# nerficg-project/faster-gaussian-splatting

Hardware: AMD Instinct MI355X
Metric: train_iters_per_sec (higher is better)
Workload: dtype f32; 1 GPU; S2: 3000000 garden-like Gaussians (SH degree 3), 1920x1080, 8 orbit views; full training iteration fwd+loss+bwd+Adam (BASELINE.json configs[2]), loss 0.8*L1+0.2*DSSIM, densification_info updated; parallelism=single GPU, n_gaussians=3000000, active_sh_bases=16, forward=one host read per pass (fgs_forward), world=1, backend=none (single process), device=cuda:0 (AMD Radeon Graphics)

## Files before the change

### faster-gaussian-splatting_amd/csrc/adam.hip

```cpp
#include "fgs_adam.h"

namespace fgs {


template <bool NT> __device__ __forceinline__ float4 load4(const float* p) { return NT ? load_float4_nt(p) : *reinterpret_cast<const float4*>(p); }
template <bool NT> __device__ __forceinline__ void store4(float* p, const float4 v) {
    if (NT) store_float4_nt(p, v);
    else *reinterpret_cast<float4*>(p) = v;
}

__device__ __forceinline__ bool adam_block_gradient_needed(const AdamArgs& a, const AdamGroup& G, const uint32_t b) {
    if (a.live_blocks[b] != 0) return true;
    return !(G.grad[(size_t)b * 64u * G.row_len] == 0.0f);
}

enum : int { kAdamSkip = 0, kAdamZero = 1, kAdamRead = 2 };
__device__ __forceinline__ int adam_piece_plan(const AdamArgs& a, const AdamGroup& G, const int64_t first, const int64_t last) {
    if (a.live_blocks == nullptr || G.row_len == 0u) return kAdamRead;
    const uint32_t r0 = static_cast<uint32_t>(first) / G.row_len, r1 = static_cast<uint32_t>(last) / G.row_len;
    const uint32_t b0 = r0 >> 6, b1 = r1 >> 6;
    const bool need0 = adam_block_gradient_needed(a, G, b0), need1 = b1 == b0 ? need0 : adam_block_gradient_needed(a, G, b1);
    if (a.quiet_blocks != nullptr) {
        const uint8_t q0 = a.quiet_blocks[b0], q1 = b1 == b0 ? q0 : a.quiet_blocks[b1];
        if (need0 && q0 != 0) a.quiet_blocks[b0] = 0;
        if (b1 != b0 && need1 && q1 != 0) a.quiet_blocks[b1] = 0;
        if (!need0 && !need1 && q0 != 0 && q1 != 0) return kAdamSkip;
    }
    return need0 || need1 ? kAdamRead : kAdamZero;
}

template <int U, bool NT>
__global__ void __launch_bounds__(256) adam_kernel(const AdamArgs a) {
    const uint32_t blk = a.reverse ? a.total_blocks - 1u - blockIdx.x : blockIdx.x;
    int gidx = 0;
#pragma unroll
    for (int j = 1; j < 8; ++j) if (j < a.n_groups && blk >= a.g[j].first_block) gidx = j;
    const AdamGroup& G = a.g[gidx];
    const int64_t block_base = (int64_t)(blk - G.first_block) * (256 * 4 * U);
    float4 g4[U];
    float4 p4[U], m4[U], v4[U];
    bool full[U], run[U];
#pragma unroll
    for (int u = 0; u < U; ++u) {
        const int64_t base = block_base + ((int64_t)u * 256 + threadIdx.x) * 4;
        full[u] = base + 4 <= G.n;
        run[u] = false;
        if (full[u]) {
            const int plan = adam_piece_plan(a, G, base, base + 3);
            run[u] = plan != kAdamSkip;
            if (run[u]) {
                g4[u] = plan == kAdamRead ? load4<NT>(G.grad + base) : make_float4(0.0f, 0.0f, 0.0f, 0.0f);
                p4[u] = load4<NT>(G.param + base); m4[u] = load4<NT>(G.exp_avg + base); v4[u] = load4<NT>(G.exp_avg_sq + base);
            }
        }
    }
#pragma unroll
    for (int u = 0; u < U; ++u) {
        const int64_t base = block_base + ((int64_t)u * 256 + threadIdx.x) * 4;
        if (full[u]) {
            if (run[u]) {
                adam_update(p4[u].x, m4[u].x, v4[u].x, g4[u].x, G.h); adam_update(p4[u].y, m4[u].y, v4[u].y, g4[u].y, G.h);
                adam_update(p4[u].z, m4[u].z, v4[u].z, g4[u].z, G.h); adam_update(p4[u].w, m4[u].w, v4[u].w, g4[u].w, G.h);
                store4<NT>(G.param + base, p4[u]); store4<NT>(G.exp_avg + base, m4[u]); store4<NT>(G.exp_avg_sq + base, v4[u]);
            }
        } else if (base < G.n) {
            const int plan = adam_piece_plan(a, G, base, G.n - 1);
            if (plan != kAdamSkip)
                adam_scalar_tail(G.param, G.exp_avg, G.exp_avg_sq, base, G.n, G.h, [&](const int64_t e) { return plan == kAdamRead ? G.grad[e] : 0.0f; });
        }
    }
}

__global__ void __launch_bounds__(256) adam_quiet_scan_kernel(const AdamQuietScanArgs a) {
    const uint32_t b = blockIdx.x;
    const uint32_t rows = min(64u, a.rows - b * 64u);
    bool zero = true;
    for (int k = 0; k < a.n_groups; ++k) {
        const size_t first = (size_t)b * 64u * a.row_len[k];
        const uint32_t len = rows * a.row_len[k];
#pragma unroll
        for (int w = 0; w < 2; ++w) {
            const float* t = (w == 0 ? a.m[k] : a.v[k]) + first;
            const uint32_t vec = (reinterpret_cast<uintptr_t>(t) & 15u) == 0 ? len >> 2 : 0u;
            for (uint32_t i = threadIdx.x; i < vec; i += 256u) {
                const float4 x = load_float4_nt(t + 4u * i);
                zero = zero && x.x == 0.0f && x.y == 0.0f && x.z == 0.0f && x.w == 0.0f;
            }
            for (uint32_t e = 4u * vec + threadIdx.x; e < len; e += 256u) zero = zero && t[e] == 0.0f;
        }
    }
    const int all_zero = __syncthreads_and(zero ? 1 : 0);
    if (threadIdx.x == 0) a.quiet_out[b] = all_zero ? 1 : 0;
}

hipError_t launch_adam_quiet_scan(const AdamQuietScanArgs& a, hipStream_t s) {
    if (a.rows == 0) return hipSuccess;
    hipLaunchKernelGGL(adam_quiet_scan_kernel, dim3((a.rows + 63u) / 64u), dim3(256), 0, s, a);
    return hipGetLastError();
}

static uint32_t assign_adam_blocks(AdamArgs& a, const int u) {
    uint32_t blocks = 0;
    for (int k = 0; k < a.n_groups; ++k) { a.g[k].first_block = blocks; blocks += static_cast<uint32_t>((a.g[k].n + 1024 * u - 1) / (1024 * u)); }
    return a.total_blocks = blocks;
}

#ifdef FGS_DEV_SWITCHES
static bool launch_adam_exhibit(const AdamArgs& a_in, hipStream_t s) {
    const int unroll_opt = g_adam_unroll, nontemporal = g_adam_nontemporal, reverse = g_adam_reverse;
    if (nontemporal && reverse) return false;
    AdamArgs a = a_in;
    a.reverse = reverse;
    const int u = nontemporal ? 1 : (unroll_opt == 2 || unroll_opt == 4 ? unroll_opt : 1);
    const uint32_t blocks = assign_adam_blocks(a, u);
    if (blocks == 0) return true;
    if (nontemporal) hipLaunchKernelGGL((adam_kernel<1, true>), dim3(blocks), dim3(256), 0, s, a);
    else if (u == 1) hipLaunchKernelGGL((adam_kernel<1, false>), dim3(blocks), dim3(256), 0, s, a);
    else if (u == 2) hipLaunchKernelGGL((adam_kernel<2, false>), dim3(blocks), dim3(256), 0, s, a);
    else hipLaunchKernelGGL((adam_kernel<4, false>), dim3(blocks), dim3(256), 0, s, a);
    return true;
}
#endif

hipError_t launch_adam(const AdamArgs& a_in, hipStream_t s) {
#ifdef FGS_DEV_SWITCHES
    if (launch_adam_exhibit(a_in, s)) return hipGetLastError();
#endif
    AdamArgs a = a_in;
    a.reverse = 1;
    const uint32_t blocks = assign_adam_blocks(a, 1);
    if (blocks == 0) return hipSuccess;
    hipLaunchKernelGGL((adam_kernel<1, true>), dim3(blocks), dim3(256), 0, s, a);
    return hipGetLastError();
}

}
```

### faster-gaussian-splatting_amd/csrc/api_debug.hip

```cpp
#include "fgs_host.h"

using namespace fgs;
extern "C" {
#pragma GCC visibility push(default)
#ifdef FGS_DEV_SWITCHES
int32_t fgs_debug_set_backward_variant(int32_t variant) {
    if (variant < 0 || variant > 5) return fail(FGS_ERR_INVALID_ARGUMENT, "variant must be 0 (systolic), 1 (strip), 2 (systolic, global dL/dC), 3 (live list + compacted pixels), 4 (lane = pixel, matrix-core reduction) or 5 (3 with the items of a wave chained through the lanes)");
    fgs::g_backward_variant = variant;
    return FGS_OK;
}

int32_t fgs_debug_set_option(int32_t key, int32_t value) {
    switch (key) {
        case 0: return fgs_debug_set_backward_variant(value);
        case 1: if (value != 1 && value != 2 && value != 4) return fail(FGS_ERR_INVALID_ARGUMENT, "adam unroll must be 1, 2 or 4");
                fgs::g_adam_unroll = value; return FGS_OK;
        case 2: fgs::g_adam_nontemporal = value ? 1 : 0; return FGS_OK;
        case 3: g_fused_single_kernel = value ? 1 : 0; return FGS_OK;
        case 7: fgs::g_backward_ablate = value & 15; return FGS_OK;
        case 13: if (value < 1) return fail(FGS_ERR_INVALID_ARGUMENT, "K11 variant 4 needs at least one workgroup"); fgs::g_k11m_max_blocks = value; return FGS_OK;
        case 8: fgs::g_adam_reverse = value ? 1 : 0; return FGS_OK;
        case 9: fgs::g_depth_sort_mode = value & 3; return FGS_OK;
        case 10: if (value < 0 || (value > 64 && (value < 251 || value > 255))) return fail(FGS_ERR_INVALID_ARGUMENT, "tile mapping must be 252 (one strip of tile columns per XCD, default), 254 (device-side block plan), 0 (bands), 255 (bands, bottom first) or 1..64 (row groups)");
                 fgs::g_tile_row_group = value; return FGS_OK;
        case 11: g_library_bucket_scan = value ? 1 : 0; return FGS_OK;
        case 12: fgs::g_plan_experiment = value & 3; return FGS_OK;
        case 14: if (value < 1) return fail(FGS_ERR_INVALID_ARGUMENT, "the chained K11 needs at least one wave"); fgs::g_k11_chain_waves = value; return FGS_OK;
        case 5: if (value < 0 || value > 32) return fail(FGS_ERR_INVALID_ARGUMENT, "seq_tiles must be 0 (flattened counting) or 1..32");
                g_seq_tiles = value; return FGS_OK;
        default: return fail(FGS_ERR_INVALID_ARGUMENT, "unknown option %d", key);
    }
}

#endif

size_t fgs_debug_radix_sort_temp_bytes(int32_t n, int32_t end_bit) {
    return n < 0 ? 0 : own_sort_temp_bytes(static_cast<uint32_t>(n), end_bit);
}

int32_t fgs_debug_radix_sort(void* keys0, void* keys1, uint32_t* vals0, uint32_t* vals1, int32_t n, int32_t key_bytes, int32_t end_bit,
                             void* temp, size_t temp_bytes, void* stream) {
    if (n < 0 || (key_bytes != 2 && key_bytes != 4) || end_bit < 1 || end_bit > 8 * key_bytes)
        return fail(FGS_ERR_INVALID_ARGUMENT, "bad sort arguments");
    if (n > 0 && (!keys0 || !keys1 || !vals0 || !vals1 || !temp)) return fail(FGS_ERR_INVALID_ARGUMENT, "NULL buffer");
    int selector = 0;
    uint32_t* vals[2] = {vals0, vals1};
    if (key_bytes == 2) {
        uint16_t* k[2] = {static_cast<uint16_t*>(keys0), static_cast<uint16_t*>(keys1)};
        FGS_HIP(own_sort_pairs_u16(temp, temp_bytes, k, vals, selector, static_cast<uint32_t>(n), end_bit, static_cast<hipStream_t>(stream)));
    } else {
        uint32_t* k[2] = {static_cast<uint32_t*>(keys0), static_cast<uint32_t*>(keys1)};
        FGS_HIP(own_sort_pairs_u32(temp, temp_bytes, k, vals, selector, static_cast<uint32_t>(n), end_bit, static_cast<hipStream_t>(stream)));
    }
    return selector;
}

int32_t fgs_debug_depth_sort(uint32_t* keys0, uint32_t* keys1, uint32_t* vals0, uint32_t* vals1, int32_t n, float near_plane, float far_plane,
                             void* temp, size_t temp_bytes, void* stream) {
    if (n < 0) return fail(FGS_ERR_INVALID_ARGUMENT, "bad sort arguments");
    if (n > 0 && (!keys0 || !keys1 || !vals0 || !vals1 || !temp)) return fail(FGS_ERR_INVALID_ARGUMENT, "NULL buffer");
    int selector = 0;
    uint32_t* k[2] = {keys0, keys1};
    uint32_t* vals[2] = {vals0, vals1};
    FGS_HIP(own_depth_sort(temp, temp_bytes, k, vals, selector, static_cast<uint32_t>(n), nullptr, depth_key_range(near_plane, far_plane),
                           static_cast<hipStream_t>(stream)));
    return selector;
}

int32_t fgs_debug_wave_selftest(uint32_t* out_device_256, void* stream) {
    if (!out_device_256) return fail(FGS_ERR_INVALID_ARGUMENT, "NULL output");
    FGS_HIP(launch_wave_selftest(out_device_256, static_cast<hipStream_t>(stream)));
    return FGS_OK;
}
#pragma GCC visibility pop
}
```

### faster-gaussian-splatting_amd/csrc/api_ops.hip

```cpp
#include "fgs_host.h"

using namespace fgs;
namespace {
struct AdcScratch {
    uint32_t* plan; uint4* offsets; uint32_t* totals; char* scan_temp; size_t scan_temp_bytes;
    static AdcScratch carve(Carver& c, uint32_t n) {
        AdcScratch b;
        b.plan = c.take<uint32_t>("plan", n);
        b.offsets = c.take<uint4>("offsets", n);
        b.totals = c.take<uint32_t>("totals", 4);
        b.scan_temp_bytes = adc_scan_temp_bytes(n);
        b.scan_temp = c.take<char>("scan_temp", b.scan_temp_bytes);
        return b;
    }
};

struct LossScratch {
    size_t plane3, partials_at;
    LossScratch(int width, int height) : plane3(3 * static_cast<size_t>(width) * static_cast<size_t>(height)), partials_at((3 * plane3 + 1) & ~static_cast<size_t>(1)) {}
    void point_maps(LossArgs& a, void* scratch) const { a.d_mu = static_cast<float*>(scratch); a.d_m11 = a.d_mu + plane3; a.d_m12 = a.d_m11 + plane3; }
};
}

extern "C" {
#pragma GCC visibility push(default)
int32_t fgs_adam_step_multi_quiet(int32_t n_groups, const float* const* grads, float* const* params, float* const* exp_avgs,
                                  float* const* exp_avg_sqs, const int64_t* n_elements, const int32_t* steps, const double* lrs,
                                  double beta1, double beta2, double eps, const uint8_t* live_blocks, const int32_t* floats_per_gaussian,
                                  uint8_t* quiet_blocks, void* stream) {
    if (n_groups < 0 || n_groups > 8) return fail(FGS_ERR_INVALID_ARGUMENT, "n_groups %d (max 8)", n_groups);
    if ((live_blocks != nullptr || quiet_blocks != nullptr) && floats_per_gaussian == nullptr) return fail(FGS_ERR_INVALID_ARGUMENT, "live_blocks / quiet_blocks without floats_per_gaussian");
    AdamArgs a{};
    a.live_blocks = live_blocks;
    uint32_t blocks = 0;
    int64_t rows = -1;
    bool quiet_ok = quiet_blocks != nullptr && live_blocks != nullptr;
    for (int k = 0; k < n_groups; ++k) {
        if (n_elements[k] < 0 || steps[k] < 1) return fail(FGS_ERR_INVALID_ARGUMENT, "group %d: n_elements / step", k);
        if (n_elements[k] == 0) continue;
        if (!grads[k] || !params[k] || !exp_avgs[k] || !exp_avg_sqs[k]) return fail(FGS_ERR_INVALID_ARGUMENT, "group %d: NULL tensor", k);
        AdamGroup& g = a.g[a.n_groups++];
        g.grad = grads[k]; g.param = params[k]; g.exp_avg = exp_avgs[k]; g.exp_avg_sq = exp_avg_sqs[k]; g.n = n_elements[k];
        g.h = adam_hyper(steps[k], lrs[k], beta1, beta2, eps);
        g.row_len = 0;
        if (live_blocks != nullptr || quiet_blocks != nullptr) {
            if (floats_per_gaussian[k] < 1 || n_elements[k] % floats_per_gaussian[k] != 0) return fail(FGS_ERR_INVALID_ARGUMENT, "group %d: floats_per_gaussian", k);
            if (n_elements[k] < (int64_t{1} << 32)) g.row_len = static_cast<uint32_t>(floats_per_gaussian[k]);
            if (quiet_blocks != nullptr) {
                const int64_t n = n_elements[k] / floats_per_gaussian[k];
                if (rows >= 0 && n != rows) return fail(FGS_ERR_INVALID_ARGUMENT, "group %d: quiet_blocks needs one N for all groups (%lld vs %lld)", k, (long long)n, (long long)rows);
                rows = n;
            }
        }
        quiet_ok = quiet_ok && g.row_len != 0u && g.h.eps > 0.0f && std::isfinite(g.h.eps) && std::isfinite(g.h.step_size) && std::isfinite(g.h.beta1) &&
                   std::isfinite(g.h.beta2) && std::isfinite(g.h.bc2_sqrt_rcp);
        g.first_block = blocks;
        blocks += static_cast<uint32_t>((n_elements[k] + 1023) / 1024);
    }
    a.total_blocks = blocks;
    if (quiet_ok) a.quiet_blocks = quiet_blocks;
    else if (quiet_blocks != nullptr && rows > 0) FGS_HIP(hipMemsetAsync(quiet_blocks, 0, static_cast<size_t>((rows + 63) / 64), static_cast<hipStream_t>(stream)));
    { StageScope t(ST_ADAM, static_cast<hipStream_t>(stream)); FGS_HIP(launch_adam(a, static_cast<hipStream_t>(stream))); }
    return FGS_OK;
}

int32_t fgs_adam_step_multi_live(int32_t n_groups, const float* const* grads, float* const* params, float* const* exp_avgs,
                                 float* const* exp_avg_sqs, const int64_t* n_elements, const int32_t* steps, const double* lrs,
                                 double beta1, double beta2, double eps, const uint8_t* live_blocks, const int32_t* floats_per_gaussian,
                                 void* stream) {
    return fgs_adam_step_multi_quiet(n_groups, grads, params, exp_avgs, exp_avg_sqs, n_elements, steps, lrs, beta1, beta2, eps, live_blocks,
                                     floats_per_gaussian, nullptr, stream);
}

int32_t fgs_adam_quiet_scan(int32_t n_groups, const float* const* exp_avgs, const float* const* exp_avg_sqs, const int64_t* n_elements,
                            const int32_t* floats_per_gaussian, uint8_t* quiet_out, void* stream) {
    if (n_groups < 0 || n_groups > 8) return fail(FGS_ERR_INVALID_ARGUMENT, "n_groups %d (max 8)", n_groups);
    if (n_groups > 0 && (!exp_avgs || !exp_avg_sqs || !n_elements || !floats_per_gaussian)) return fail(FGS_ERR_INVALID_ARGUMENT, "NULL argument");
    AdamQuietScanArgs a{};
    int64_t rows = -1;
    for (int k = 0; k < n_groups; ++k) {
        if (n_elements[k] < 0 || floats_per_gaussian[k] < 1 || n_elements[k] % floats_per_gaussian[k] != 0) return fail(FGS_ERR_INVALID_ARGUMENT, "group %d: n_elements / floats_per_gaussian", k);
        const int64_t n = n_elements[k] / floats_per_gaussian[k];
        if (rows >= 0 && n != rows) return fail(FGS_ERR_INVALID_ARGUMENT, "group %d: all groups must have the same N (%lld vs %lld)", k, (long long)n, (long long)rows);
        rows = n;
        if (n > 0x7fffffff || floats_per_gaussian[k] > (1 << 20)) return fail(FGS_ERR_INVALID_ARGUMENT, "group %d: N / floats_per_gaussian out of range", k);
        if (n == 0) continue;
        if (!exp_avgs[k] || !exp_avg_sqs[k]) return fail(FGS_ERR_INVALID_ARGUMENT, "group %d: NULL tensor", k);
        a.m[a.n_groups] = exp_avgs[k]; a.v[a.n_groups] = exp_avg_sqs[k]; a.row_len[a.n_groups] = static_cast<uint32_t>(floats_per_gaussian[k]);
        ++a.n_groups;
    }
    if (rows <= 0) return FGS_OK;
    if (!quiet_out) return fail(FGS_ERR_INVALID_ARGUMENT, "NULL quiet_out");
    a.rows = static_cast<uint32_t>(rows); a.quiet_out = quiet_out;
    FGS_HIP(launch_adam_quiet_scan(a, static_cast<hipStream_t>(stream)));
    return FGS_OK;
}

int32_t fgs_adam_step_multi(int32_t n_groups, const float* const* grads, float* const* params, float* const* exp_avgs,
                            float* const* exp_avg_sqs, const int64_t* n_elements, const int32_t* steps, const double* lrs,
                            double beta1, double beta2, double eps, void* stream) {
    return fgs_adam_step_multi_live(n_groups, grads, params, exp_avgs, exp_avg_sqs, n_elements, steps, lrs, beta1, beta2, eps, nullptr, nullptr, stream);
}

int32_t fgs_adam_step(const float* grad, float* param, float* exp_avg, float* exp_avg_sq, int64_t n_elements,
                      int32_t step, double lr, double beta1, double beta2, double eps, void* stream) {
    return fgs_adam_step_multi(1, &grad, &param, &exp_avg, &exp_avg_sq, &n_elements, &step, &lr, beta1, beta2, eps, stream);
}

int32_t fgs_update_3d_filter(const float* positions, const float* w2c, float* filter_3d, uint8_t* visibility_mask, int32_t n_points,
                             int32_t width, int32_t height, float focal_x, float focal_y, float center_x, float center_y,
                             float near_plane, float clipping_tolerance, float distance2filter, void* stream) {
    if (n_points < 0 || (n_points > 0 && (!positions || !w2c || !filter_3d || !visibility_mask))) return fail(FGS_ERR_INVALID_ARGUMENT, "bad argument");
    const float bounds_factor = clipping_tolerance + 0.5f;
    const float width_f = static_cast<float>(width), height_f = static_cast<float>(height);
    const float max_x = bounds_factor * width_f, max_y = bounds_factor * height_f;
    const float off_x = center_x - 0.5f * width_f, off_y = center_y - 0.5f * height_f;
    const float left = (-max_x - off_x) / focal_x, right = (max_x - off_x) / focal_x;
    const float top = (-max_y - off_y) / focal_y, bottom = (max_y - off_y) / focal_y;
    FGS_HIP(launch_update_3d_filter(positions, w2c, filter_3d, visibility_mask, n_points, left, right, top, bottom, near_plane,
                                    distance2filter, static_cast<hipStream_t>(stream)));
    return FGS_OK;
}

int32_t fgs_relocation_table(float* table_host_2500) {
    if (!table_host_2500) return fail(FGS_ERR_INVALID_ARGUMENT, "NULL table");
    relocation_coefficients(table_host_2500);
    return FGS_OK;
}

int32_t fgs_relocation_adjustment(const float* old_opacities, const float* old_scales, const int64_t* n_samples_per_primitive,
                                  const float* table_device, float* new_opacities, float* new_scales, int32_t n_primitives, void* stream) {
    if (n_primitives < 0 || (n_primitives > 0 && (!old_opacities || !old_scales || !n_samples_per_primitive || !table_device || !new_opacities || !new_scales)))
        return fail(FGS_ERR_INVALID_ARGUMENT, "bad argument");
    FGS_HIP(launch_relocation(old_opacities, old_scales, n_samples_per_primitive, table_device, new_opacities, new_scales,
                              static_cast<unsigned>(n_primitives), static_cast<hipStream_t>(stream)));
    return FGS_OK;
}

int32_t fgs_add_noise(const float* raw_scales, const float* raw_rotations, const float* raw_opacities, const float* random_samples,
                      float* means, int32_t n_primitives, float current_lr, void* stream) {
    if (n_primitives < 0 || (n_primitives > 0 && (!raw_scales || !raw_rotations || !raw_opacities || !random_samples || !means)))
        return fail(FGS_ERR_INVALID_ARGUMENT, "bad argument");
    FGS_HIP(launch_add_noise(raw_scales, raw_rotations, raw_opacities, random_samples, means, static_cast<unsigned>(n_primitives), current_lr,
                             static_cast<hipStream_t>(stream)));
    return FGS_OK;
}

size_t fgs_adc_scratch_bytes(int32_t n_primitives) {
    if (n_primitives < 0) return 0;
    Carver c(nullptr);
    AdcScratch::carve(c, static_cast<uint32_t>(n_primitives));
    return c.total();
}

int32_t fgs_adc_plan(const float* densification_info, const float* scales, const float* rotations, const float* opacities, int32_t n_primitives,
                     float grad_threshold, float min_opacity, int32_t prune_large_gaussians, float percent_dense, float extent,
                     void* scratch, int32_t* counts_out, void* stream_) {
    if (n_primitives < 0 || !counts_out || !scratch) return fail(FGS_ERR_INVALID_ARGUMENT, "bad argument");
    if (n_primitives > 0 && (!densification_info || !scales || !rotations || !opacities)) return fail(FGS_ERR_INVALID_ARGUMENT, "NULL tensor");
    if (!(min_opacity > 0.0f && min_opacity < 1.0f) || !(percent_dense * extent > 0.0f)) return fail(FGS_ERR_INVALID_ARGUMENT, "min_opacity / percent_dense * extent out of range");
    hipStream_t stream = static_cast<hipStream_t>(stream_);
    Carver c(scratch);
    const AdcScratch sc = AdcScratch::carve(c, static_cast<uint32_t>(n_primitives));
    AdcPlanArgs a{};
    a.densification_info = densification_info; a.scales = scales; a.rotations = rotations; a.opacities = opacities;
    a.n = static_cast<uint32_t>(n_primitives);
    a.grad_threshold = grad_threshold;
    a.min_opacity_logit = static_cast<float>(std::log(static_cast<double>(min_opacity) / (1.0 - static_cast<double>(min_opacity))));
    a.log_small = static_cast<float>(std::log(static_cast<double>(percent_dense) * static_cast<double>(extent)));
    a.log_large = static_cast<float>(std::log(0.1 * static_cast<double>(extent)));
    a.prune_large = prune_large_gaussians ? 1 : 0;
    a.plan = sc.plan; a.offsets = sc.offsets; a.totals = sc.totals; a.scan_temp = sc.scan_temp; a.scan_temp_bytes = sc.scan_temp_bytes;
    FGS_HIP(launch_adc_plan(a, stream));
    uint32_t host[4] = {0, 0, 0, 0};
    FGS_HIP(hipMemcpyAsync(host, sc.totals, sizeof(host), hipMemcpyDeviceToHost, stream));
    FGS_HIP(hipStreamSynchronize(stream));
    for (int k = 0; k < 4; ++k) counts_out[k] = static_cast<int32_t>(host[k]);
    return FGS_OK;
}

int32_t fgs_adc_apply(const float* const* params, const float* const* exp_avgs, const float* const* exp_avg_sqs,
                      float* const* out_params, float* const* out_exp_avgs, float* const* out_exp_avg_sqs,
                      const float* noise, const void* scratch, int32_t n_primitives, int32_t total_sh_bases_rest, void* stream_) {
    if (n_primitives < 0 || !params || !out_params || !scratch || total_sh_bases_rest < 0) return fail(FGS_ERR_INVALID_ARGUMENT, "bad argument");
    if ((exp_avgs == nullptr) != (exp_avg_sqs == nullptr) || (exp_avgs && (!out_exp_avgs || !out_exp_avg_sqs))) return fail(FGS_ERR_INVALID_ARGUMENT, "moments: all four arrays or none");
    if (n_primitives == 0) return FGS_OK;
    hipStream_t stream = static_cast<hipStream_t>(stream_);
    Carver c(const_cast<void*>(scratch));
    const AdcScratch sc = AdcScratch::carve(c, static_cast<uint32_t>(n_primitives));
    const uint32_t width[6] = {3u, 3u, 3u * static_cast<uint32_t>(total_sh_bases_rest), 1u, 3u, 4u};
    const int kind[6] = {1, 0, 0, 0, 2, 0};
    for (int k = 0; k < 6; ++k) {
        if (width[k] == 0) continue;
        if (!params[k] || !out_params[k]) return fail(FGS_ERR_INVALID_ARGUMENT, "NULL tensor in group %d", k);
        AdcScatterArgs a{};
        a.in_p = params[k]; a.out_p = out_params[k];
        if (exp_avgs && exp_avgs[k]) {
            if (!exp_avg_sqs[k] || !out_exp_avgs[k] || !out_exp_avg_sqs[k]) return fail(FGS_ERR_INVALID_ARGUMENT, "NULL moment tensor in group %d", k);
            a.in_m = exp_avgs[k]; a.in_v = exp_avg_sqs[k]; a.out_m = out_exp_avgs[k]; a.out_v = out_exp_avg_sqs[k];
        }
        a.scales = params[4]; a.rotations = params[5]; a.noise = noise;
        a.plan = sc.plan; a.offsets = sc.offsets; a.totals = sc.totals;
        a.n = static_cast<uint32_t>(n_primitives); a.width = width[k];
        FGS_HIP(launch_adc_scatter(kind[k], a, stream));
    }
    return FGS_OK;
}

int32_t fgs_gather_rows(int32_t n_tensors, const float* const* in, float* const* out, const int32_t* widths, const int64_t* index,
                        int32_t n_rows, void* stream) {
    if (n_tensors < 0 || n_tensors > kGatherTensors || n_rows < 0) return fail(FGS_ERR_INVALID_ARGUMENT, "n_tensors %d (max %d) / n_rows %d", n_tensors, kGatherTensors, n_rows);
    if (n_rows == 0 || n_tensors == 0) return FGS_OK;
    if (!in || !out || !widths || !index) return fail(FGS_ERR_INVALID_ARGUMENT, "NULL argument");
    GatherArgs a{};
    for (int k = 0; k < n_tensors; ++k) {
        if (widths[k] < 0) return fail(FGS_ERR_INVALID_ARGUMENT, "tensor %d: width %d", k, widths[k]);
        if (widths[k] == 0) continue;
        if (!in[k] || !out[k]) return fail(FGS_ERR_INVALID_ARGUMENT, "tensor %d: NULL", k);
        GatherTensor& t = a.t[a.n_tensors++];
        t.in = in[k]; t.out = out[k]; t.width = static_cast<uint32_t>(widths[k]);
    }
    a.n_rows = static_cast<uint32_t>(n_rows); a.index = index;
    FGS_HIP(launch_gather_rows(a, static_cast<hipStream_t>(stream)));
    return FGS_OK;
}

size_t fgs_morton_order_temp_bytes(int32_t n_points) { return n_points < 0 ? 0 : morton_temp_bytes(static_cast<uint32_t>(n_points)); }

int32_t fgs_morton_order(const float* means, const float* lo, const float* hi, int64_t* order_out, int32_t n_points, void* temp, size_t temp_bytes,
                         void* stream) {
    if (n_points < 0) return fail(FGS_ERR_INVALID_ARGUMENT, "n_points %d", n_points);
    if (n_points == 0) return FGS_OK;
    if (!means || !lo || !hi || !order_out || !temp || temp_bytes < morton_temp_bytes(static_cast<uint32_t>(n_points))) return fail(FGS_ERR_INVALID_ARGUMENT, "NULL / short buffer");
    FGS_HIP(run_morton_order(means, lo, hi, order_out, static_cast<uint32_t>(n_points), temp, temp_bytes, static_cast<hipStream_t>(stream)));
    return FGS_OK;
}

size_t fgs_l1_dssim_scratch_bytes(int32_t width, int32_t height) {
    if (width <= 0 || height <= 0) return 0;
    return sizeof(float) * (LossScratch(width, height).partials_at + l1_dssim_partials(width, height));
}

int32_t fgs_l1_dssim_loss(const float* image, const float* target, int32_t width, int32_t height, float lambda_l1, float lambda_dssim,
                          float* sums, float* grad_image, void* scratch, void* stream_) {
    if (!image || !target || !sums || !scratch || width <= 0 || height <= 0) return fail(FGS_ERR_INVALID_ARGUMENT, "bad argument");
    hipStream_t stream = static_cast<hipStream_t>(stream_);
    LossArgs a{};
    a.image = image; a.target = target; a.sums = sums; a.grad = grad_image;
    const LossScratch layout(width, height);
    layout.point_maps(a, scratch); a.partials = a.d_mu + layout.partials_at;
    if ((reinterpret_cast<uintptr_t>(a.partials) & 7u) != 0) return fail(FGS_ERR_INVALID_ARGUMENT, "scratch must be 8-byte aligned");
    a.width = width; a.height = height; a.lambda_l1 = lambda_l1; a.lambda_dssim = lambda_dssim;
    { StageScope t(ST_LOSS, stream); FGS_HIP(launch_l1_dssim(a, stream)); }
    return FGS_OK;
}

int32_t fgs_l1_dssim_backward(const float* image, const float* target, int32_t width, int32_t height, float lambda_l1, float lambda_dssim,
                              const float* upstream, float* grad_image, const void* scratch, void* stream_) {
    if (!image || !target || !grad_image || !scratch || width <= 0 || height <= 0) return fail(FGS_ERR_INVALID_ARGUMENT, "bad argument");
    hipStream_t stream = static_cast<hipStream_t>(stream_);
    LossArgs a{};
    a.image = image; a.target = target; a.grad = grad_image; a.upstream = upstream;
    LossScratch(width, height).point_maps(a, const_cast<void*>(scratch));
    a.width = width; a.height = height; a.lambda_l1 = lambda_l1; a.lambda_dssim = lambda_dssim;
    { StageScope t(ST_LOSS, stream); FGS_HIP(launch_l1_dssim_backward(a, stream)); }
    return FGS_OK;
}
#pragma GCC visibility pop
}
```

### faster-gaussian-splatting_amd/csrc/fgs_kernels.h

```cpp
#pragma once
#include <hip/hip_runtime.h>
#include <atomic>
#include <cmath>
#include <cstddef>
#include <cstdint>
#include "fgs_config.h"
#include "fgs_math.h"

namespace fgs {

struct PreprocessArgs {
    const float* means; const float* scales; const float* rotations; const float* opacities;
    const float* sh0; const float* sh_rest;
    PrimRec* rec; uint32_t* n_touched;
    uint32_t* depth_keys; uint32_t* prim_idx;
    uint4* foot;
    uint32_t* counters;
    uint32_t* huge_list;
    uint32_t* hot_list;
    uint2* ranges; uint32_t n_tiles;
    float* acc;
    uint32_t n;
    int seq_tiles;
    int count_appended;
    CameraArgs cam;
};
hipError_t launch_preprocess(bool inference, const PreprocessArgs& a, hipStream_t s);
struct PreprocessBatch { int n_views; PreprocessArgs v[kMaxBatchViews]; };
hipError_t launch_preprocess_batch(const PreprocessBatch& b, hipStream_t s);

struct DepthKeyRange { uint32_t base; int bits; };
DepthKeyRange depth_key_range(float near_plane, float far_plane);
size_t depth_sort_temp_bytes(uint32_t n);
hipError_t run_depth_sort(void* temp, size_t temp_bytes, uint32_t* keys[2], uint32_t* vals[2], int& selector, uint32_t n_visible,
                          const uint32_t* n_visible_ptr, DepthKeyRange range, uint4* foot[2], uint32_t* tile_counts,
                          uint32_t* big_list, uint32_t* big_count, hipStream_t s);
hipError_t launch_tile_count_sums(const uint32_t* tile_counts, uint32_t* wave_sums, uint32_t* block_sums,
                                  uint32_t n_visible, const uint32_t* n_visible_ptr, hipStream_t s);

size_t tile_sort_temp_bytes(uint32_t n_instances, int key_bytes, int end_bit);
hipError_t launch_create_instances(int key_bytes, const uint4* foot_sorted, const uint32_t* wave_sums,
                                   const uint32_t* block_sums, uint32_t* offsets,
                                   const PrimRec* rec, void* inst_keys, uint32_t* inst_prims, uint32_t grid_w, uint32_t n_visible,
                                   const uint32_t* n_visible_ptr, uint32_t capacity, uint32_t* counters,
                                   const uint32_t* big_list, const uint32_t* big_count, hipStream_t s);
hipError_t run_tile_sort(void* temp, size_t temp_bytes, int key_bytes, void* keys[2], uint32_t* vals[2], int& selector,
                         uint32_t n_instances, const uint32_t* n_instances_ptr, int end_bit, hipStream_t s);
hipError_t launch_extract_ranges(int key_bytes, const void* sorted_keys, uint2* ranges, uint32_t n_instances, const uint32_t* n_instances_ptr, hipStream_t s);

#ifdef FGS_DEV_SWITCHES
#define FGS_SWITCH(name, value) inline std::atomic<int> name{value}
#else
#define FGS_SWITCH(name, value) constexpr int name = (value)
#endif
constexpr unsigned kColumnsTopDown = 252u, kColumnsBottomUp = 251u;
constexpr unsigned kPlannedBlocks = 254u;
constexpr unsigned kBandsThroughPlan = 253u;
#ifdef FGS_DEV_SWITCHES
FGS_SWITCH(g_tile_row_group, static_cast<int>(kColumnsTopDown));
FGS_SWITCH(g_library_bucket_scan, 0);
FGS_SWITCH(g_plan_experiment, 0);
FGS_SWITCH(g_k11_chain_waves, 4096);
FGS_SWITCH(g_seq_tiles, kSeqTiles);
FGS_SWITCH(g_depth_sort_mode, 1);
FGS_SWITCH(g_adam_reverse, 1);
FGS_SWITCH(g_adam_nontemporal, 1);
FGS_SWITCH(g_adam_unroll, 1);
#endif
FGS_SWITCH(g_fused_single_kernel, 1);
size_t own_sort_temp_bytes(uint32_t n, int end_bit);
struct SortPayload { const uint4* rows_in; uint4* rows_out; uint32_t* count_out; int iota_values;
                     uint32_t* big_list; uint32_t* big_count; };
hipError_t own_depth_sort(void* temp, size_t temp_bytes, uint32_t* keys[2], uint32_t* vals[2], int& selector, uint32_t n, const uint32_t* n_ptr,
                          DepthKeyRange range, hipStream_t s, const SortPayload* payload = nullptr);
#ifdef FGS_DEV_SWITCHES
bool depth_sort_exhibit(hipError_t& result, void* temp, size_t temp_bytes, uint32_t* keys[2], uint32_t* vals[2], int& selector, uint32_t n,
                        const uint32_t* n_ptr, DepthKeyRange range, hipStream_t s, const SortPayload* payload);
#endif
hipError_t own_sort_pairs_u32(void* temp, size_t temp_bytes, uint32_t* keys[2], uint32_t* vals[2], int& selector, uint32_t n, int end_bit, hipStream_t s);
hipError_t own_sort_pairs_u16(void* temp, size_t temp_bytes, uint16_t* keys[2], uint32_t* vals[2], int& selector, uint32_t n, int end_bit, hipStream_t s);
hipError_t own_sort_pairs_u32_device_count(void* temp, size_t temp_bytes, uint32_t* keys[2], uint32_t* vals[2], int& selector, uint32_t capacity,
                                           const uint32_t* n_ptr, int end_bit, hipStream_t s);
hipError_t own_sort_pairs_u16_device_count(void* temp, size_t temp_bytes, uint16_t* keys[2], uint32_t* vals[2], int& selector, uint32_t capacity,
                                           const uint32_t* n_ptr, int end_bit, hipStream_t s);

hipError_t launch_plan_tiles(const uint2* ranges, uint32_t* bucket_offsets, uint32_t* tile_plan, uint32_t n_tiles, uint32_t grid_w, uint32_t grid_h,
                             hipStream_t s);
#ifdef FGS_DEV_SWITCHES
hipError_t launch_plan_tiles_exhibit(const uint2* ranges, uint32_t* bucket_offsets, uint32_t* tile_plan, uint32_t n_tiles, uint32_t grid_w, uint32_t grid_h,
                                     hipStream_t s);
size_t bucket_scan_temp_bytes(uint32_t n_tiles);
hipError_t run_bucket_scan(void* temp, size_t temp_bytes, const uint2* ranges, uint32_t* bucket_offsets, uint32_t n_tiles, hipStream_t s);
#endif

struct BlendArgs {
    const uint2* ranges; const uint32_t* bucket_offsets; const uint32_t* inst_prims; const PrimRec* rec;
    const float* bg; float* image;
    float* final_T; uint32_t* n_processed; uint32_t* max_n_processed;
    uint32_t* bucket_tile; float4* ckpt;
    uint32_t width, height, grid_w, n_tiles;
    uint32_t row_group;
    const uint32_t* tile_plan;
    uint32_t grid_h;
    int to_chw, clamp_output;
    float* scores;
    const float* means; const float* w2c;
    float* aux_alpha; float* aux_depth; float* aux_median;
};
hipError_t launch_blend(bool training, const BlendArgs& a, hipStream_t s);
hipError_t launch_blend_aux(const BlendArgs& a, hipStream_t s);
hipError_t launch_pruning_scores(const BlendArgs& a, hipStream_t s);
struct BlendDepthArgs { BlendArgs blend; float* ckpt_d; };
hipError_t launch_blend_training_aux(const BlendDepthArgs& a, hipStream_t s);

struct BlendBackwardArgs {
    const uint2* ranges; const uint32_t* bucket_offsets; const uint32_t* inst_prims; const PrimRec* rec;
    const float* bg; const float* grad_image; const float* image;
    const float* final_T; const uint32_t* n_processed; const uint32_t* max_n_processed;
    const uint32_t* bucket_tile; const float4* ckpt;
    float4* pixrec;
    float* acc;
    float* acc_hot;
    const uint32_t* hot_list; const uint32_t* hot_count;
    uint2* work_list; uint32_t* live_count;
    uint32_t* live_offsets;
    uint32_t n, width, height, grid_w, n_tiles, n_buckets_cap;
    uint32_t clear_all_f4, clear_hot_f4; int clear_everything;
    uint32_t* dirty_flag;
    int proper_aa;
    int ablate;
    int variant;
};
hipError_t launch_stage_pixels(const BlendBackwardArgs& a, hipStream_t s);
hipError_t launch_blend_backward(const BlendBackwardArgs& a, hipStream_t s);
struct BlendDepthPart {
    const float* grad_alpha; const float* grad_depth;
    const float* depth;
    const float* ckpt_d;
    float4* pixaux;
    const float* means; const float* w2c;
    float* acc_z;
    float* acc_z_hot;
    uint32_t clear_z_f4;
};
struct BlendBackwardDepthArgs { BlendBackwardArgs blend; BlendDepthPart d; };
hipError_t launch_stage_pixels_depth(const BlendBackwardDepthArgs& a, hipStream_t s);
hipError_t launch_blend_backward_depth(const BlendBackwardDepthArgs& a, hipStream_t s);
hipError_t launch_depth_mean_gradient(const float* acc_z, const uint32_t* n_touched, const float* w2c, float* grad_means, uint32_t n, hipStream_t s);
struct BlendAbsPart {
    float* acc_abs;
    float* acc_abs_hot;
    uint32_t clear_abs_f4;
};
struct BlendBackwardAbsArgs { BlendBackwardArgs blend; BlendAbsPart abs; };
struct BlendBackwardDepthAbsArgs { BlendBackwardArgs blend; BlendDepthPart d; BlendAbsPart abs; };
hipError_t launch_stage_pixels_abs(const BlendBackwardAbsArgs& a, hipStream_t s);
hipError_t launch_blend_backward_abs(const BlendBackwardAbsArgs& a, hipStream_t s);
hipError_t launch_stage_pixels_depth_abs(const BlendBackwardDepthAbsArgs& a, hipStream_t s);
hipError_t launch_blend_backward_depth_abs(const BlendBackwardDepthAbsArgs& a, hipStream_t s);
hipError_t launch_abs_densification(const float* acc_abs, const uint32_t* n_touched, float* info, uint32_t n, float width, float height, hipStream_t s);

constexpr int kMaxFeatureChannels = 64;
struct FeatureBlendArgs {
    const uint2* ranges; const uint32_t* inst_prims; const PrimRec* rec;
    const uint32_t* n_processed; const uint32_t* max_n_processed;
    const float* features;
    float* feature_map;
    const float* feature_map_in;
    const float* grad_feature_map;
    float* grad_features;
    float* acc;
    uint32_t n_channels, width, height, grid_w, grid_h, n_tiles;
    int proper_aa, detach_geometry;
};
hipError_t launch_blend_features(const FeatureBlendArgs& a, hipStream_t s);
hipError_t launch_blend_features_backward(const FeatureBlendArgs& a, hipStream_t s);

struct AdamHyper { float step_size, beta1, beta2, eps, bc2_sqrt_rcp; };

struct BackwardView {
    CameraArgs cam;
    const uint32_t* n_touched;
    const float* acc;
    const uint32_t* slot;
    float* view_dir;
    const float* acc_z;
};
struct PreprocessBackwardArgs {
    const float* means; const float* scales; const float* rotations; const float* opacities; const float* sh_rest;
    float* grad_means; float* grad_scales; float* grad_rotations; float* grad_opacities; float* grad_sh0;
    float* densification_info;
    uint32_t n;
    int accumulate;
    int n_views; BackwardView view[kMaxBatchViews];
    float* p[5]; float* m[5]; float* v[5]; AdamHyper h[5];
    uint8_t* live_blocks;
    uint8_t* reached_blocks;
    const uint8_t* prior_blocks;
    int vector_ok;
};
hipError_t launch_preprocess_backward(bool fused_adam, const PreprocessBackwardArgs& a, hipStream_t s);

struct ShRestView { const float* view_dir; const uint32_t* n_touched; const float* acc; const uint32_t* slot; };
struct ShRestArgs {
    int n_views; ShRestView view[kMaxBatchViews];
    float* grad_sh_rest;
    float* p; float* m; float* v; AdamHyper h;
    uint32_t n; uint32_t total_sh_rest; uint32_t active_sh_bases;
    int accumulate;
};
hipError_t launch_sh_rest_backward(bool fused_adam, const ShRestArgs& a, hipStream_t s);
hipError_t launch_fused_backward_adam(const PreprocessBackwardArgs& a, const ShRestArgs& sh, hipStream_t s);
hipError_t launch_backward_gradients(const PreprocessBackwardArgs& a, const ShRestArgs& sh, hipStream_t s);
constexpr int kPoseTerms = 15;
constexpr int kPoseLineFloats = 16;
constexpr uint32_t kPoseMaxChunks = 128;
struct PosePart {
    float* partials;
    double* chunk_sums;
    float* grad_w2c; float* grad_cam_position;
};
struct PreprocessBackwardPoseArgs { PreprocessBackwardArgs k12; PosePart pose; };
hipError_t launch_backward_gradients_pose(const PreprocessBackwardArgs& a, const ShRestArgs& sh, const PosePart& pose, hipStream_t s);

struct AdamGroup { const float* grad; float* param; float* exp_avg; float* exp_avg_sq; int64_t n; AdamHyper h; uint32_t first_block;
                   uint32_t row_len; };
struct AdamArgs { AdamGroup g[8]; int n_groups; uint32_t total_blocks; int reverse; const uint8_t* live_blocks; uint8_t* quiet_blocks; };
hipError_t launch_adam(const AdamArgs& a, hipStream_t s);
struct AdamQuietScanArgs { const float* m[8]; const float* v[8]; uint32_t row_len[8]; int n_groups; uint32_t rows; uint8_t* quiet_out; };
hipError_t launch_adam_quiet_scan(const AdamQuietScanArgs& a, hipStream_t s);

struct LossArgs {
    const float* image; const float* target;
    float* sums;
    float* grad;
    float* d_mu; float* d_m11; float* d_m12;
    float* partials;
    int width, height;
    float lambda_l1, lambda_dssim;
    const float* upstream;
};
size_t l1_dssim_partials(int width, int height);
hipError_t launch_l1_dssim(const LossArgs& a, hipStream_t s);
hipError_t launch_l1_dssim_backward(const LossArgs& a, hipStream_t s);

struct PackRecordsView { const PrimRec* rec; const uint32_t* n_touched; const uint32_t* depth_keys; const uint32_t* prim_idx;
                         const uint32_t* counters; uint32_t* slot; uint32_t* out; uint32_t* counts_out; };
struct PackRecordsBatch { int n_views; uint32_t capacity; PackRecordsView v[kMaxBatchViews]; };
hipError_t launch_pack_splat_records(const PackRecordsBatch& b, hipStream_t s);
struct ShardOrder { int n_shards; uint32_t count[kMaxBatchViews]; };
hipError_t launch_unpack_splat_records(const uint32_t* records, uint32_t n, PrimRec* rec, uint32_t* n_touched, uint32_t* depth_keys,
                                       uint32_t* prim_idx, uint4* foot, uint2* ranges, uint32_t n_tiles, uint32_t* hot_list, uint32_t* hot_count, const ShardOrder& order,
                                       hipStream_t s);
hipError_t launch_pack_acc(const float* acc, uint32_t n, float* out, const ShardOrder& order, hipStream_t s);

hipError_t launch_update_3d_filter(const float* positions, const float* w2c, float* filter_3d, uint8_t* visibility_mask, int n,
                                   float left, float right, float top, float bottom, float near_plane, float distance2filter, hipStream_t s);
void relocation_coefficients(float* out );
hipError_t launch_relocation(const float* old_opacities, const float* old_scales, const int64_t* n_samples, const float* table_device,
                             float* new_opacities, float* new_scales, unsigned n, hipStream_t s);
hipError_t launch_add_noise(const float* raw_scales, const float* raw_rotations, const float* raw_opacities, const float* random_samples,
                            float* means, unsigned n, float current_lr, hipStream_t s);

struct AdcPlanArgs {
    const float* densification_info;
    const float* scales; const float* rotations; const float* opacities;
    uint32_t n;
    float grad_threshold, min_opacity_logit, log_small, log_large; int prune_large;
    uint32_t* plan; uint4* offsets; uint32_t* totals;
    void* scan_temp; size_t scan_temp_bytes;
};
size_t adc_scan_temp_bytes(uint32_t n);
hipError_t launch_adc_plan(const AdcPlanArgs& a, hipStream_t s);
struct AdcScatterArgs {
    const float* in_p; const float* in_m; const float* in_v;
    float* out_p; float* out_m; float* out_v;
    const float* scales; const float* rotations; const float* noise;
    const uint32_t* plan; const uint4* offsets; const uint32_t* totals;
    uint32_t n, width;
};
hipError_t launch_adc_scatter(int kind, const AdcScatterArgs& a, hipStream_t s);
constexpr int kGatherTensors = 18;
struct GatherTensor { const float* in; float* out; uint32_t width; uint32_t first_block; };
struct GatherArgs { GatherTensor t[kGatherTensors]; int n_tensors; uint32_t n_rows; const int64_t* index; };
hipError_t launch_gather_rows(const GatherArgs& a, hipStream_t s);
size_t morton_temp_bytes(uint32_t n);
hipError_t run_morton_order(const float* means, const float* lo, const float* hi, int64_t* order_out, uint32_t n, void* temp, size_t temp_bytes, hipStream_t s);

#ifdef FGS_DEV_SWITCHES
extern std::atomic<int> g_backward_ablate;
extern std::atomic<int> g_k11m_max_blocks;
extern std::atomic<int> g_backward_variant;
void launch_blend_backward_exhibit(const BlendBackwardArgs& a, hipStream_t s);
#endif
int blend_backward_variant();
hipError_t launch_wave_selftest(uint32_t* out , hipStream_t s);

}
```

Before: 693.1 iters/s (1 view each, whole job).

## Process Adam in 4-piece chunks per block with shared per-block skip plans

The default Adam launch now uses 4 float4 pieces per thread (4096 floats per chunk) instead of 1. Each workgroup first evaluates the live/quiet plan for the 64-row blocks it covers into shared memory and exits early if all are skippable. A software-prefetch loop over span chunks is added, with span defaulting to 1. The goal is fewer workgroups, fewer redundant global reads of the live/quiet flags, and more memory-level parallelism per thread. The cost is more registers per thread, which may lower occupancy.

Measured after the change: 711.4 iters/s (1 view each, whole job) (median of 6 runs). 1.03x the previous value.

```diff
diff --git a/faster-gaussian-splatting_amd/csrc/adam.hip b/faster-gaussian-splatting_amd/csrc/adam.hip
--- a/faster-gaussian-splatting_amd/csrc/adam.hip
+++ b/faster-gaussian-splatting_amd/csrc/adam.hip
@@ -15,59 +15,92 @@
 }
 
 enum : int { kAdamSkip = 0, kAdamZero = 1, kAdamRead = 2 };
-__device__ __forceinline__ int adam_piece_plan(const AdamArgs& a, const AdamGroup& G, const int64_t first, const int64_t last) {
-    if (a.live_blocks == nullptr || G.row_len == 0u) return kAdamRead;
-    const uint32_t r0 = static_cast<uint32_t>(first) / G.row_len, r1 = static_cast<uint32_t>(last) / G.row_len;
-    const uint32_t b0 = r0 >> 6, b1 = r1 >> 6;
-    const bool need0 = adam_block_gradient_needed(a, G, b0), need1 = b1 == b0 ? need0 : adam_block_gradient_needed(a, G, b1);
+__device__ __forceinline__ int adam_block_plan(const AdamArgs& a, const AdamGroup& G, const uint32_t b) {
+    const bool need = adam_block_gradient_needed(a, G, b);
     if (a.quiet_blocks != nullptr) {
-        const uint8_t q0 = a.quiet_blocks[b0], q1 = b1 == b0 ? q0 : a.quiet_blocks[b1];
-        if (need0 && q0 != 0) a.quiet_blocks[b0] = 0;
-        if (b1 != b0 && need1 && q1 != 0) a.quiet_blocks[b1] = 0;
-        if (!need0 && !need1 && q0 != 0 && q1 != 0) return kAdamSkip;
+        const uint8_t q = a.quiet_blocks[b];
+        if (need && q != 0) a.quiet_blocks[b] = 0;
+        if (!need && q != 0) return kAdamSkip;
     }
-    return need0 || need1 ? kAdamRead : kAdamZero;
+    return need ? kAdamRead : kAdamZero;
 }
+
+__device__ __forceinline__ int adam_piece_plan(const uint8_t* plans, const uint32_t b_first, const uint32_t row_len, const int64_t first, const int64_t last) {
+    const uint32_t b0 = ((static_cast<uint32_t>(first) / row_len) >> 6) - b_first, b1 = ((static_cast<uint32_t>(last) / row_len) >> 6) - b_first;
+    const int p0 = plans[b0];
+    return b1 == b0 ? p0 : max(p0, static_cast<int>(plans[b1]));
+}
+
+constexpr uint32_t kAdamMaxSpan = 32;
+constexpr int kAdamPieces = 4;
+
+constexpr int kAdamNotFull = -1;
+template <int U> struct AdamChunk { float4 g[U], p[U], m[U], v[U]; int plan[U]; };
 
 template <int U, bool NT>
 __global__ void __launch_bounds__(256) adam_kernel(const AdamArgs a) {
+    __shared__ uint8_t plans[kAdamMaxSpan * 16 * U];
     const uint32_t blk = a.reverse ? a.total_blocks - 1u - blockIdx.x : blockIdx.x;
     int gidx = 0;
 #pragma unroll
     for (int j = 1; j < 8; ++j) if (j < a.n_groups && blk >= a.g[j].first_block) gidx = j;
     const AdamGroup& G = a.g[gidx];
-    const int64_t block_base = (int64_t)(blk - G.first_block) * (256 * 4 * U);
-    float4 g4[U];
-    float4 p4[U], m4[U], v4[U];
-    bool full[U], run[U];
+    constexpr int64_t kChunk = 256 * 4 * U;
+    const int64_t span_first = (int64_t)(blk - G.first_block) * a.span * kChunk;
+    const int64_t span_end = min(G.n, span_first + (int64_t)a.span * kChunk);
+    const bool flagged = a.live_blocks != nullptr && G.row_len != 0u;
+    uint32_t b_first = 0;
+    if (flagged) {
+        b_first = (static_cast<uint32_t>(span_first) / G.row_len) >> 6;
+        const uint32_t b_last = (static_cast<uint32_t>(span_end - 1) / G.row_len) >> 6;
+        bool idle = true;
+        for (uint32_t b = b_first + threadIdx.x; b <= b_last; b += 256u) {
+            const int plan = adam_block_plan(a, G, b);
+            plans[b - b_first] = static_cast<uint8_t>(plan);
+            idle = idle && plan == kAdamSkip;
+        }
+        if (__syncthreads_and(idle ? 1 : 0)) return;
+    }
+    const int chunks = static_cast<int>((span_end - span_first + kChunk - 1) / kChunk);
+    const auto chunk_base = [&](const int c) { return span_first + (int64_t)(a.reverse ? chunks - 1 - c : c) * kChunk; };
+    const auto request = [&](const int64_t chunk, AdamChunk<U>& r) {
 #pragma unroll
-    for (int u = 0; u < U; ++u) {
-        const int64_t base = block_base + ((int64_t)u * 256 + threadIdx.x) * 4;
-        full[u] = base + 4 <= G.n;
-        run[u] = false;
-        if (full[u]) {
-            const int plan = adam_piece_plan(a, G, base, base + 3);
-            run[u] = plan != kAdamSkip;
-            if (run[u]) {
-                g4[u] = plan == kAdamRead ? load4<NT>(G.grad + base) : make_float4(0.0f, 0.0f, 0.0f, 0.0f);
-                p4[u] = load4<NT>(G.param + base); m4[u] = load4<NT>(G.exp_avg + base); v4[u] = load4<NT>(G.exp_avg_sq + base);
+        for (int u = 0; u < U; ++u) {
+            const int64_t base = chunk + ((int64_t)u * 256 + threadIdx.x) * 4;
+            r.plan[u] = kAdamNotFull;
+            if (base + 4 <= G.n) {
+                const int plan = flagged ? adam_piece_plan(plans, b_first, G.row_len, base, base + 3) : kAdamRead;
+                r.plan[u] = plan;
+                if (plan != kAdamSkip) {
+                    r.g[u] = plan == kAdamRead ? load4<NT>(G.grad + base) : make_float4(0.0f, 0.0f, 0.0f, 0.0f);
+                    r.p[u] = load4<NT>(G.param + base); r.m[u] = load4<NT>(G.exp_avg + base); r.v[u] = load4<NT>(G.exp_avg_sq + base);
+                }
             }
         }
-    }
+    };
+    const auto finish = [&](const int64_t chunk, AdamChunk<U>& r) {
 #pragma unroll
-    for (int u = 0; u < U; ++u) {
-        const int64_t base = block_base + ((int64_t)u * 256 + threadIdx.x) * 4;
-        if (full[u]) {
-            if (run[u]) {
-                adam_update(p4[u].x, m4[u].x, v4[u].x, g4[u].x, G.h); adam_update(p4[u].y, m4[u].y, v4[u].y, g4[u].y, G.h);
-                adam_update(p4[u].z, m4[u].z, v4[u].z, g4[u].z, G.h); adam_update(p4[u].w, m4[u].w, v4[u].w, g4[u].w, G.h);
-                store4<NT>(G.param + base, p4[u]); store4<NT>(G.exp_avg + base, m4[u]); store4<NT>(G.exp_avg_sq + base, v4[u]);
+        for (int u = 0; u < U; ++u) {
+            const int64_t base = chunk + ((int64_t)u * 256 + threadIdx.x) * 4;
+            if (r.plan[u] != kAdamNotFull) {
+                if (r.plan[u] != kAdamSkip) {
+                    adam_update(r.p[u].x, r.m[u].x, r.v[u].x, r.g[u].x, G.h); adam_update(r.p[u].y, r.m[u].y, r.v[u].y, r.g[u].y, G.h);
+                    adam_update(r.p[u].z, r.m[u].z, r.v[u].z, r.g[u].z, G.h); adam_update(r.p[u].w, r.m[u].w, r.v[u].w, r.g[u].w, G.h);
+                    store4<NT>(G.param + base, r.p[u]); store4<NT>(G.exp_avg + base, r.m[u]); store4<NT>(G.exp_avg_sq + base, r.v[u]);
+                }
+            } else if (base < G.n) {
+                const int plan = flagged ? adam_piece_plan(plans, b_first, G.row_len, base, G.n - 1) : kAdamRead;
+                if (plan != kAdamSkip)
+                    adam_scalar_tail(G.param, G.exp_avg, G.exp_avg_sq, base, G.n, G.h, [&](const int64_t e) { return plan == kAdamRead ? G.grad[e] : 0.0f; });
             }
-        } else if (base < G.n) {
-            const int plan = adam_piece_plan(a, G, base, G.n - 1);
-            if (plan != kAdamSkip)
-                adam_scalar_tail(G.param, G.exp_avg, G.exp_avg_sq, base, G.n, G.h, [&](const int64_t e) { return plan == kAdamRead ? G.grad[e] : 0.0f; });
         }
+    };
+    AdamChunk<U> cur;
+    int64_t chunk = chunk_base(0);
+    request(chunk, cur);
+    for (int c = 0; c < chunks; ++c) {
+        finish(chunk, cur);
+        if (c + 1 < chunks) request(chunk = chunk_base(c + 1), cur);
     }
 }
 
@@ -100,8 +133,10 @@
 }
 
 static uint32_t assign_adam_blocks(AdamArgs& a, const int u) {
+    a.span = min(max(static_cast<uint32_t>(g_adam_span), 1u), kAdamMaxSpan);
+    const int64_t span_floats = (int64_t)a.span * 1024 * u;
     uint32_t blocks = 0;
-    for (int k = 0; k < a.n_groups; ++k) { a.g[k].first_block = blocks; blocks += static_cast<uint32_t>((a.g[k].n + 1024 * u - 1) / (1024 * u)); }
+    for (int k = 0; k < a.n_groups; ++k) { a.g[k].first_block = blocks; blocks += static_cast<uint32_t>((a.g[k].n + span_floats - 1) / span_floats); }
     return a.total_blocks = blocks;
 }
 
@@ -128,9 +163,9 @@
 #endif
     AdamArgs a = a_in;
     a.reverse = 1;
-    const uint32_t blocks = assign_adam_blocks(a, 1);
+    const uint32_t blocks = assign_adam_blocks(a, kAdamPieces);
     if (blocks == 0) return hipSuccess;
-    hipLaunchKernelGGL((adam_kernel<1, true>), dim3(blocks), dim3(256), 0, s, a);
+    hipLaunchKernelGGL((adam_kernel<kAdamPieces, true>), dim3(blocks), dim3(256), 0, s, a);
     return hipGetLastError();
 }
 
diff --git a/faster-gaussian-splatting_amd/csrc/api_debug.hip b/faster-gaussian-splatting_amd/csrc/api_debug.hip
--- a/faster-gaussian-splatting_amd/csrc/api_debug.hip
+++ b/faster-gaussian-splatting_amd/csrc/api_debug.hip
@@ -26,6 +26,8 @@
         case 11: g_library_bucket_scan = value ? 1 : 0; return FGS_OK;
         case 12: fgs::g_plan_experiment = value & 3; return FGS_OK;
         case 14: if (value < 1) return fail(FGS_ERR_INVALID_ARGUMENT, "the chained K11 needs at least one wave"); fgs::g_k11_chain_waves = value; return FGS_OK;
+        case 15: if (value < 1 || value > 32) return fail(FGS_ERR_INVALID_ARGUMENT, "the Adam span must be 1..32 chunks of 1024 floats");
+                 fgs::g_adam_span = value; return FGS_OK;
         case 5: if (value < 0 || value > 32) return fail(FGS_ERR_INVALID_ARGUMENT, "seq_tiles must be 0 (flattened counting) or 1..32");
                 g_seq_tiles = value; return FGS_OK;
         default: return fail(FGS_ERR_INVALID_ARGUMENT, "unknown option %d", key);
diff --git a/faster-gaussian-splatting_amd/csrc/api_ops.hip b/faster-gaussian-splatting_amd/csrc/api_ops.hip
--- a/faster-gaussian-splatting_amd/csrc/api_ops.hip
+++ b/faster-gaussian-splatting_amd/csrc/api_ops.hip
@@ -32,7 +32,6 @@
     if ((live_blocks != nullptr || quiet_blocks != nullptr) && floats_per_gaussian == nullptr) return fail(FGS_ERR_INVALID_ARGUMENT, "live_blocks / quiet_blocks without floats_per_gaussian");
     AdamArgs a{};
     a.live_blocks = live_blocks;
-    uint32_t blocks = 0;
     int64_t rows = -1;
     bool quiet_ok = quiet_blocks != nullptr && live_blocks != nullptr;
     for (int k = 0; k < n_groups; ++k) {
@@ -54,10 +53,7 @@
         }
         quiet_ok = quiet_ok && g.row_len != 0u && g.h.eps > 0.0f && std::isfinite(g.h.eps) && std::isfinite(g.h.step_size) && std::isfinite(g.h.beta1) &&
                    std::isfinite(g.h.beta2) && std::isfinite(g.h.bc2_sqrt_rcp);
-        g.first_block = blocks;
-        blocks += static_cast<uint32_t>((n_elements[k] + 1023) / 1024);
-    }
-    a.total_blocks = blocks;
+    }
     if (quiet_ok) a.quiet_blocks = quiet_blocks;
     else if (quiet_blocks != nullptr && rows > 0) FGS_HIP(hipMemsetAsync(quiet_blocks, 0, static_cast<size_t>((rows + 63) / 64), static_cast<hipStream_t>(stream)));
     { StageScope t(ST_ADAM, static_cast<hipStream_t>(stream)); FGS_HIP(launch_adam(a, static_cast<hipStream_t>(stream))); }
diff --git a/faster-gaussian-splatting_amd/csrc/fgs_kernels.h b/faster-gaussian-splatting_amd/csrc/fgs_kernels.h
--- a/faster-gaussian-splatting_amd/csrc/fgs_kernels.h
+++ b/faster-gaussian-splatting_amd/csrc/fgs_kernels.h
@@ -68,6 +68,7 @@
 FGS_SWITCH(g_adam_unroll, 1);
 #endif
 FGS_SWITCH(g_fused_single_kernel, 1);
+FGS_SWITCH(g_adam_span, 1);
 size_t own_sort_temp_bytes(uint32_t n, int end_bit);
 struct SortPayload { const uint4* rows_in; uint4* rows_out; uint32_t* count_out; int iota_values;
                      uint32_t* big_list; uint32_t* big_count; };
@@ -225,7 +226,7 @@
 
 struct AdamGroup { const float* grad; float* param; float* exp_avg; float* exp_avg_sq; int64_t n; AdamHyper h; uint32_t first_block;
                    uint32_t row_len; };
-struct AdamArgs { AdamGroup g[8]; int n_groups; uint32_t total_blocks; int reverse; const uint8_t* live_blocks; uint8_t* quiet_blocks; };
+struct AdamArgs { AdamGroup g[8]; int n_groups; uint32_t total_blocks; int reverse; const uint8_t* live_blocks; uint8_t* quiet_blocks; uint32_t span; };
 hipError_t launch_adam(const AdamArgs& a, hipStream_t s);
 struct AdamQuietScanArgs { const float* m[8]; const float* v[8]; uint32_t row_len[8]; int n_groups; uint32_t rows; uint8_t* quiet_out; };
 hipError_t launch_adam_quiet_scan(const AdamQuietScanArgs& a, hipStream_t s);
```
